# df07/mcp-raytracer

Hardware: AMD Instinct MI355X
Metric: Msamples/sec (w×h×spp/s) Cornell 800×800 spp=256 @1/2/4/8 GPU (higher is better)
Workload: dtype f64

## Files before the change

mcp-raytracer_amd/csrc/pt_kernel.hpp:

```cpp
#pragma once

#include <hip/hip_runtime.h>

#include <cstdint>
#include <type_traits>

#include "rt_math.hpp"
#include "scene.hpp"

namespace rt {

struct DevScene {
    const RtTNode* __restrict__ tnodes;
    const RtPrim* __restrict__ prims;
    const RtPrim* __restrict__ gprims;
    const RtPre* __restrict__ gpre;
    int32_t n_pre;
    const RtExact* __restrict__ xrec;
    int32_t off_xrec;
    const int32_t* __restrict__ tprims;
    const float4* __restrict__ tsph;
    const RtMat* __restrict__ mats;
    const RtLight* __restrict__ lights;
    const RtLight* __restrict__ glights;
// ... 962 lines not shown
    struct W {
        u4 a, b;
    } w{w0, w1};
    return __builtin_bit_cast(RtExact, w);
}
template <class Real>
__device__ __forceinline__ bool prim_exact_rec(const RtExact& x, const RtPrim& p, const RayK<Real>& r, Real& t) {
    const Real inf = (Real)__builtin_inf();
    const int code = x.kind & 7;
    const bool sph = code == PRE_SPHERE;
    if (code == PRE_OTHER) return prim_exact<Real>(p, r, t);
    const Real s0 = (Real)x.s0;
    Real num, den, halfB = (Real)0, sq = (Real)0;
    float o1 = 0.f, d1 = 0.f, o2 = 0.f, d2 = 0.f;
    if (sph) {
        const V3 c = V3{x.f[0], x.f[1], x.f[2]};
        const V3 oc = sub(r.o, c);
        halfB = dot<Real>(oc, r.d);
        const Real cc = len2<Real>(oc) - s0 * s0;
        const Real disc = halfB * halfB - r.a * cc;
        if (disc < (Real)0) return false;
        sq = m_sqrt(disc);
        num = -halfB - sq;
        den = r.a;
    } else {
        const int a = (int)((aquad_axes(0) >> (2 * code)) & 3u);
        const int ia = (int)((aquad_axes(1) >> (2 * code)) & 3u);
        const int ib = (int)((aquad_axes(2) >> (2 * code)) & 3u);
        const V3 o3 = r.o, d3 = r.d;
        const float oa = sel3(o3.x, o3.y, o3.z, a), da = sel3(d3.x, d3.y, d3.z, a);
        o1 = sel3(o3.x, o3.y, o3.z, ia);
        d1 = sel3(d3.x, d3.y, d3.z, ia);
        o2 = sel3(o3.x, o3.y, o3.z, ib);
        d2 = sel3(d3.x, d3.y, d3.z, ib);
        if (!(::isfinite(o1) && ::isfinite(d1) && ::isfinite(o2) && ::isfinite(d2))) return false;
        const Real na = (x.kind & kExactNegNa) ? (Real)-1 : (Real)1;
        den = na * (Real)da;
        if (m_abs(den) < (Real)1e-8) return false;
        num = s0 - na * (Real)oa;
    }
    Real q = num / den;
    if (sph) {
        if (!(K<Real>::TMIN < q && q < inf)) {
            q = (-halfB + sq) / r.a;
            if (!(K<Real>::TMIN < q && q < inf)) return false;
        }
    } else {
        if (!(K<Real>::TMIN < q && q < inf)) return false;
        const float ph1 = (o1 + (float)((Real)d1 * q)) - x.f[0];
        const float ph2 = (o2 + (float)((Real)d2 * q)) - x.f[1];
        const Real sw = (Real)x.f[2];
        const Real alpha = sw * (Real)(ph1 * x.f[3]);
        const Real beta = sw * (Real)(ph2 * x.f[4]);
        if (alpha < (Real)0 || alpha > (Real)1 || beta < (Real)0 || beta > (Real)1) return false;
    }
    t = q;
    return true;
}

constexpr float kEt = 1e-6f;
constexpr float kWin = 0.5f + 1e-4f + 1e-6f;
struct QuadPreRay {
    float c1, c0;
};
__device__ __forceinline__ QuadPreRay quad_pre_ray(const FRay& f) {
    RT_FP32_FUSED
    return QuadPreRay{(kEt + kRel) * f.dn, kRel * f.on + 1e-30f * f.dn};
}
template <int CODE>
__device__ __forceinline__ bool aquad_maybe_pre(const float* v, const FRay& f, const QuadPreRay& qr, float& lo) {
    RT_FP32_FUSED
    constexpr int a = (CODE - 1) % 3, vflag = (CODE - 1) / 3;
    constexpr int ia = vflag ? (a + 1) % 3 : (a + 2) % 3, ib = vflag ? (a + 2) % 3 : (a + 1) % 3;
    const float xa = v[0], sv = v[1], su = v[2], nq1 = v[3], nq2 = v[4], qk = v[5];
    lo = kTminLo;
    if (!(::fabsf(f.d[a]) > f.pthr)) return true;
    const float t = __builtin_fmaf(xa, f.inv[a], f.noi[a]);
    const float tn = ::fabsf(t) + ::fabsf(f.noi[a]);
    const float et = __builtin_fmaf(kEt, tn, 1e-30f);
    if (t + et < kTminLo) return false;
    lo = t - et;
    const float alpha = __builtin_fmaf(__builtin_fmaf(t, f.d[ia], f.o[ia]), sv, nq1);
    const float beta = __builtin_fmaf(__builtin_fmaf(t, f.d[ib], f.o[ib]), su, nq2);
    const float dp = __builtin_fmaf(tn, qr.c1, qr.c0 + qk);
    const float wa = __builtin_fmaf(-::fabsf(sv), dp, ::fabsf(alpha));
    const float wb = __builtin_fmaf(-::fabsf(su), dp, ::fabsf(beta));
    return !(wa > kWin) && !(wb > kWin);
}


__device__ __forceinline__ void sphere_maybe2(const float* v, const FRay& f, bool& m0, bool& m1, float& lo0,
                                              float& lo1) {
    RT_FP32_FUSED
    const pf2 cx = {v[0], v[1]}, cy = {v[2], v[3]}, cz = {v[4], v[5]}, r = {v[6], v[7]}, rr = {v[8], v[9]};
    const pf2 ox = pf2_of(f.o[0]) - cx, oy = pf2_of(f.o[1]) - cy, oz = pf2_of(f.o[2]) - cz;
    const pf2 b = pf2_fma(oz, pf2_of(f.d[2]), pf2_fma(oy, pf2_of(f.d[1]), ox * pf2_of(f.d[0])));
    const pf2 oo = pf2_fma(oz, oz, pf2_fma(oy, oy, ox * ox));
    const pf2 disc = pf2_fma(b, b, -(pf2_of(f.a) * (oo - rr)));
    const pf2 tol = pf2_fma(pf2_of(4.0f * kRel * f.a), oo + rr, pf2_of(1e-30f));
    const pf2 dt = __builtin_elementwise_max(disc, pf2_of(0.0f)) + tol;
    const pf2 sq = pf2{__builtin_amdgcn_sqrtf(dt.x), __builtin_amdgcn_sqrtf(dt.y)} * pf2_of(1.0f + kRel);
    const pf2 e0 = pf2_fma(pf2_of(3.0f), sq, pf2_fma(pf2_of(f.dn), r, pf2_of(2.0f) * pf2_abs(b)));
    const pf2 et = pf2_fma(e0, pf2_of(kRel * f.ia), pf2_of(1e-30f));
    const pf2 far = pf2_fma((sq - b) * pf2_of(f.ia), pf2_of(1.0f + kRel), et);
    const pf2 r1 = (-b - sq) * pf2_of(f.ia);
    const pf2 lo = pf2_fma(-pf2_abs(r1), pf2_of(kRel), r1) - et;
    m0 = !(disc.x < -tol.x) && !(far.x < kTminLo);
    m1 = !(disc.y < -tol.y) && !(far.y < kTminLo);
    lo0 = lo.x;
    lo1 = lo.y;
}

template <int CODE>
__device__ __forceinline__ void aquad_maybe_pre2(const float* v, const FRay& f, const QuadPreRay& qr, bool& m0,
                                                 bool& m1, float& lo0, float& lo1) {
    RT_FP32_FUSED
    constexpr int a = (CODE - 1) % 3, vflag = (CODE - 1) / 3;
    constexpr int ia = vflag ? (a + 1) % 3 : (a + 2) % 3, ib = vflag ? (a + 2) % 3 : (a + 1) % 3;
    const pf2 xa = {v[0], v[1]}, sv = {v[2], v[3]}, su = {v[4], v[5]}, nq1 = {v[6], v[7]}, nq2 = {v[8], v[9]};
    const pf2 nsv = {v[10], v[11]}, nsu = {v[12], v[13]};
    const float qk = v[14];
    const pf2 t = pf2_fma(xa, pf2_of(f.inv[a]), pf2_of(f.noi[a]));
    const float an = ::fabsf(f.noi[a]);
    const pf2 tn = {::fabsf(t.x) + an, ::fabsf(t.y) + an};
    const pf2 et = pf2_fma(pf2_of(kEt), tn, pf2_of(1e-30f));
    const pf2 te = t + et;
    const pf2 lo = t - et;
    const pf2 alpha = pf2_fma(pf2_fma(t, pf2_of(f.d[ia]), pf2_of(f.o[ia])), sv, nq1);
    const pf2 beta = pf2_fma(pf2_fma(t, pf2_of(f.d[ib]), pf2_of(f.o[ib])), su, nq2);
    const pf2 dp = pf2_fma(tn, pf2_of(qr.c1), pf2_of(qr.c0 + qk));
    const pf2 wa = pf2_fma(nsv, dp, pf2_abs(alpha));
    const pf2 wb = pf2_fma(nsu, dp, pf2_abs(beta));
    const bool par = !(::fabsf(f.d[a]) > f.pthr);
    m0 = par || (!(te.x < kTminLo) && !(wa.x > kWin) && !(wb.x > kWin));
    m1 = par || (!(te.y < kTminLo) && !(wa.y > kWin) && !(wb.y > kWin));
    lo0 = par ? kTminLo : lo.x;
    lo1 = par ? kTminLo : lo.y;
}

__device__ __forceinline__ float lot_clamp(float lo) { return lo > 0.0f ? lo : 0.0f; }
__device__ __forceinline__ uint16_t lot_store(float lo) {
    const auto h = __builtin_amdgcn_cvt_pkrtz(lot_clamp(lo), 0.0f);
    return __builtin_bit_cast(uint16_t, h[0]);
}
__device__ __forceinline__ float lot_load(uint16_t b) { return (float)__builtin_bit_cast(_Float16, b); }
template <class SK>
__device__ __forceinline__ uint16_t* lot_column(SK* stk) {
    return reinterpret_cast<uint16_t*>(stk - threadIdx.x) + threadIdx.x;
}

struct NoHook {
    __device__ void operator()() const {}
};
template <class Real, bool COUNT, class Next>
__device__ __forceinline__ int brute_nearest_first(const DevScene& S, const RayK<Real>& r, uint32_t mask, Real& t_hit,
                                                   uint32_t* cnt, Next next) {
    Real best_t = (Real)__builtin_inf();
    int best = -1;
    float thi = __builtin_inff();
    int n_exact = 0;
    if (COUNT) {
        cnt[CT_CAND0] += mask == 0u ? 1u : 0u;
        cnt[CT_CAND2] += __popc(mask) >= 2 ? 1u : 0u;
    }
    while (mask != 0u) {
        int kb;
        float lb;
        next(mask, kb, lb);
        if (lb > thi) break;
        mask &= ~(1u << kb);
        if (COUNT) {
            count_exact(cnt);
            if (++n_exact == 2) cnt[CT_EXACT2]++;
        }
        Real t;
        const bool hit = sizeof(Real) == 8
                             ? prim_exact_rec<Real>(xrec_load(S.xrec + kb), S.prims[kb], r, t)
                             : prim_exact_rec<Real>(xrec_load(S.xrec + kb), S.prims[kb], ray_at_use<Real>(r), t);
        if (hit && (t < best_t || (t == best_t && kb < best))) {
            best_t = t;
            best = kb;
            thi = upper_f<Real>(t);
        }
    }
    t_hit = best_t;
    return best;
}

template <class Real, bool COUNT>
__device__ __forceinline__ int closest_hit_primary(const DevScene& S, const RayK<Real>& r, Real& t_hit, uint2 rec,
                                                   uint32_t* cnt) {
    const int near = (int)((rec.x >> 16) & 15u);
    const float bn = lot_load((uint16_t)rec.y), bo = lot_load((uint16_t)(rec.y >> 16));
    return brute_nearest_first<Real, COUNT>(S, r, rec.x & 0xffffu, t_hit, cnt, [&](uint32_t m, int& kb, float& lb) {
        const bool n = ((m >> near) & 1u) != 0u;
        kb = n ? near : __builtin_ctz(m);
        lb = n ? bn : bo;
    });
}

template <class Real, bool COUNT, class Hook = NoHook>
__device__ __forceinline__ int closest_hit_brute_nf(const DevScene& S, int n_prims, const RayK<Real>& r, Real& t_hit,
                                                    uint16_t* lot, uint32_t* cnt, Hook after_prefilter = Hook()) {
    (void)n_prims;
    const FRay f = make_fray(r.o, r.d);
    const QuadPreRay qr = quad_pre_ray(f);
    uint32_t mask = 0u;
    for (int g = 0; g < S.n_pre; ++g) {
        const RtPre q = ld_uniform(S.gpre, g);
        const int kind = q.head & 0xff, k0 = (q.head >> 8) & 0xff, k1 = q.head >> 16;
        const float* v = q.f;
        if (kind >= PRE_SPHERE2) {
            bool m0, m1;
            float lo0, lo1;
            if (kind == PRE_SPHERE2) {
                if (COUNT) cnt[CT_SPHERE] += 2;
                sphere_maybe2(v, f, m0, m1, lo0, lo1);
            } else {
                if (COUNT) cnt[CT_QUAD] += 2;
                switch (kind - PRE_QUAD2) {
                    case 1: aquad_maybe_pre2<1>(v, f, qr, m0, m1, lo0, lo1); break;
                    case 2: aquad_maybe_pre2<2>(v, f, qr, m0, m1, lo0, lo1); break;
                    case 3: aquad_maybe_pre2<3>(v, f, qr, m0, m1, lo0, lo1); break;
                    case 4: aquad_maybe_pre2<4>(v, f, qr, m0, m1, lo0, lo1); break;
                    case 5: aquad_maybe_pre2<5>(v, f, qr, m0, m1, lo0, lo1); break;
                    default: aquad_maybe_pre2<6>(v, f, qr, m0, m1, lo0, lo1); break;
                }
            }
            const uint32_t hw = __builtin_bit_cast(uint32_t, __builtin_amdgcn_cvt_pkrtz(lot_clamp(lo0), lot_clamp(lo1)));
            if (m0) {
                lot[k0 * kStackStride] = (uint16_t)hw;
                mask |= 1u << k0;
            }
            if (m1) {
                lot[k1 * kStackStride] = (uint16_t)(hw >> 16);
                mask |= 1u << k1;
            }
            continue;
        }
        float lo;
        bool maybe;
        if (kind == PRE_SPHERE) {
            if (COUNT) cnt[CT_SPHERE]++;
            maybe = sphere_maybe(make_float4(v[0], v[1], v[2], v[3]), f, __builtin_inff(), lo);
        } else if (kind != PRE_OTHER) {
            if (COUNT) cnt[CT_QUAD]++;
            switch (kind) {
                case 1: maybe = aquad_maybe_pre<1>(v, f, qr, lo); break;
                case 2: maybe = aquad_maybe_pre<2>(v, f, qr, lo); break;
                case 3: maybe = aquad_maybe_pre<3>(v, f, qr, lo); break;
                case 4: maybe = aquad_maybe_pre<4>(v, f, qr, lo); break;
                case 5: maybe = aquad_maybe_pre<5>(v, f, qr, lo); break;
                default: maybe = aquad_maybe_pre<6>(v, f, qr, lo); break;
            }
        } else {
            maybe = prim_maybe<COUNT>(ld_uniform(S.gprims, k0), f, lo, cnt);
        }
        if (maybe) {
            lot[k0 * kStackStride] = lot_store(lo);
            mask |= 1u << k0;
        }
    }
    after_prefilter();
    return brute_nearest_first<Real, COUNT>(S, r, mask, t_hit, cnt, [&](uint32_t rest, int& kb, float& lb) {
        kb = __builtin_ctz(rest);
        lb = lot_load(lot[kb * kStackStride]);
        for (uint32_t m = rest & (rest - 1u); m != 0u; m &= m - 1u) {
            const int k = __builtin_ctz(m);
            const float l = lot_load(lot[k * kStackStride]);
            if (l < lb) {
                lb = l;
                kb = k;
            }
        }
    });
}

struct Onb {
    V3 u, v, w;
};
template <class Real>
__device__ __forceinline__ Onb make_onb(V3 n) {
    Onb b;
    b.w = unit<Real>(n);
    const V3 a = m_abs((Real)b.w.x) > (Real)0.9 ? v3(0, 1, 0) : v3(1, 0, 0);
    b.v = unit<Real>(cross<Real>(b.w, a));
    b.u = cross<Real>(b.w, b.v);
    return b;
}
template <class Real>
__device__ __forceinline__ V3 onb_local(const Onb& b, V3 a) {
    return add(add(scale<Real>(b.u, (Real)a.x), scale<Real>(b.v, (Real)a.y)), scale<Real>(b.w, (Real)a.z));
}

template <class Real>
__device__ __forceinline__ V3 random_in_unit_sphere(uint64_t& rng) {
    while (true) {
        const Real x = (Real)-1 + (Real)2 * uniform<Real>(rng);
        const Real y = (Real)-1 + (Real)2 * uniform<Real>(rng);
        const Real z = (Real)-1 + (Real)2 * uniform<Real>(rng);
        const V3 p = mk<Real>(x, y, z);
        if (len2<Real>(p) < (Real)1) return p;
    }
}

template <class Real>
__device__ __forceinline__ V3 dielectric_dir(Real ior, bool front, V3 din, V3 n, uint64_t& rng, bool& reflected) {
    const Real ratio = front ? ((Real)1 / ior) : ior;
    const V3 ud = unit<Real>(din);
    const Real cosT = js_min<Real>(dot<Real>(neg(ud), n), (Real)1);
    const Real sinT = m_sqrt((Real)1 - cosT * cosT);
    const bool cannot = ratio * sinT > (Real)1;
    bool refl = cannot;
    if (!refl) {
        Real r0 = ((Real)1 - ratio) / ((Real)1 + ratio);
        r0 = r0 * r0;
        const Real reflectance = r0 + ((Real)1 - r0) * pow5((Real)1 - cosT);
        refl = reflectance > uniform<Real>(rng);
    }
    reflected = refl;
    if (refl) return reflect<Real>(ud, n);
    const V3 perp = scale<Real>(add(ud, scale<Real>(n, cosT)), ratio);
    const V3 par = scale<Real>(n, -m_sqrt(m_abs((Real)1 - len2<Real>(perp))));
    return add(perp, par);
}

enum ScatterKind { SC_NONE = 0, SC_SPEC = 1, SC_PDF = 2 };

template <class Real>
__device__ __forceinline__ int scatter(const DevScene& S, int mi, V3 din, V3 n, bool front, uint64_t& rng, V3& att,
                                       V3& dir, int* pdf_mat = nullptr) {
    while (true) {
        const RtMat m = S.mats[mi];
        switch (m.type) {
            case MAT_LAMBERT:
                att = ld3(m.color);
                if (pdf_mat) *pdf_mat = mi;
                return SC_PDF;
            case MAT_METAL: {
                const V3 refl = reflect<Real>(unit<Real>(din), n);
                const Real fuzz = (Real)m.p0;
                V3 f = refl;
                if (fuzz > (Real)0) f = add(refl, scale<Real>(random_in_unit_sphere<Real>(rng), fuzz));
                if (dot<Real>(f, n) <= (Real)0) return SC_NONE;
                att = ld3(m.color);
                dir = f;
                return SC_SPEC;
            }
            case MAT_GLASS: {
                bool r;
                dir = dielectric_dir<Real>((Real)m.p0, front, din, n, rng, r);
                att = v3(1, 1, 1);
                return SC_SPEC;
            }
            case MAT_MIXED:
                mi = uniform<Real>(rng) < (Real)m.p0 ? m.c0 : m.c1;
                continue;
            case MAT_LAYERED: {
                bool r;
                const V3 d2 = dielectric_dir<Real>((Real)S.mats[m.c0].p0, front, din, n, rng, r);
                if (r) {
                    att = v3(1, 1, 1);
                    dir = d2;
                    return SC_SPEC;
                }
                din = d2;
                mi = m.c1;
                continue;
            }
            default:
                return SC_NONE;
        }
    }
}

template <class Real, bool COUNT, bool UNIFORM = false>
__device__ __forceinline__ Real light_pdf_value(const DevScene& S, const RtLight& L, V3 origin, V3 dir,
                                                uint32_t* cnt) {
    const RtPrim p = UNIFORM ? ld_uniform(S.gprims, L.prim) : S.prims[L.prim];
    const RayK<Real> r = make_ray<Real>(origin, dir);
    Real t;
    if (L.type == PRIM_QUAD) {
        if (COUNT) cnt[CT_LIGHT_QUAD]++;
        const int code = aquad_code(p);
        const bool hit = code != 0 ? aquad_t<Real>(p, code, origin, dir, K<Real>::TMIN, (Real)__builtin_inf(), t)
                                   : planar_t<Real, true>(p, r, K<Real>::TMIN, (Real)__builtin_inf(), t);
        if (!hit) return (Real)0;
        const V3 hp = ray_at<Real>(origin, dir, t);
        const V3 n = ld3(p.g3);
        const bool front = dot<Real>(dir, n) <= (Real)0;
        const V3 hn = front ? n : neg(n);
        const Real d2 = len2<Real>(sub(hp, origin));
        const Real cosine = m_abs(dot<Real>(dir, hn));
        return d2 / ((Real)L.area * cosine);
    }
    if (COUNT) cnt[CT_LIGHT_SPHERE]++;
    if (!sphere_t<Real>(p, r, K<Real>::TMIN, (Real)__builtin_inf(), t)) return (Real)0;
    const Real rad = sphere_radius<Real>(p);
    const Real d2 = len2<Real>(sub(ld3(p.g0), origin));
    if (d2 <= rad * rad) return (Real)1 / ((Real)4 * K<Real>::PI);
    const Real cosT = m_sqrt((Real)1 - rad * rad / d2);
    const Real solid = (Real)2 * K<Real>::PI * ((Real)1 - cosT);
    return (Real)1 / solid;
}

template <class Real>
__device__ __forceinline__ V3 light_generate(const DevScene& S, const RtLight& L, V3 origin, uint64_t& rng) {
    const RtPrim p = S.prims[L.prim];
    if (L.type == PRIM_QUAD) {
        const Real alpha = uniform<Real>(rng);
        const Real beta = uniform<Real>(rng);
        const V3 rp = add(add(ld3(p.g0), scale<Real>(ld3(p.g1), alpha)), scale<Real>(ld3(p.g2), beta));
        return unit<Real>(sub(rp, origin));
    }
    const V3 oc = sub(ld3(p.g0), origin);
    const Real d2 = len2<Real>(oc);
    const Onb b = make_onb<Real>(oc);
    const Real rad = sphere_radius<Real>(p);
    const Real r1 = uniform<Real>(rng);
    const Real r2 = uniform<Real>(rng);
    const Real z = (Real)1 + r2 * (m_sqrt((Real)1 - rad * rad / d2) - (Real)1);
    const Real phi = (Real)2 * K<Real>::PI * r1;
    const Real s = m_sqrt((Real)1 - z * z);
    Real sn, cs;
    m_sincos(phi, sn, cs);
    return onb_local<Real>(b, mk<Real>(cs * s, sn * s, z));
}

__device__ __forceinline__ double div_pi(double x) {
    constexpr double kPi = 3.141592653589793, kInvPi = 1.0 / 3.141592653589793;
    const double q = x * kInvPi;
    const double r = __builtin_fma(-q, kPi, x);
    return __builtin_fma(r, kInvPi, q);
}
__device__ __forceinline__ float div_pi(float x) { return x / K<float>::PI; }

template <class Real>
__device__ __forceinline__ Real cosine_value(const Onb& b, V3 dir) {
    const Real c = dot<Real>(unit<Real>(dir), b.w);
    return c <= (Real)0 ? (Real)0 : div_pi(c);
}

__device__ __forceinline__ uint8_t to_u8(float c) {
    const double r = ::sqrt((double)c);
    const double v = ::floor(255.999 * r);
    if (!(v > 0.0)) return 0;
    if (v >= 255.0) return 255;
    return (uint8_t)v;
}

__device__ __forceinline__ unsigned long long wave_sum(unsigned long long v) {
#pragma unroll
    for (int o = 32; o > 0; o >>= 1) v += __shfl_xor(v, o, 64);
    return v;
}
__device__ __forceinline__ unsigned long long wave_min(unsigned long long v) {
#pragma unroll
    for (int o = 32; o > 0; o >>= 1) { unsigned long long x = __shfl_xor(v, o, 64); v = x < v ? x : v; }
    return v;
}
__device__ __forceinline__ unsigned long long wave_max(unsigned long long v) {
#pragma unroll
    for (int o = 32; o > 0; o >>= 1) { unsigned long long x = __shfl_xor(v, o, 64); v = x > v ? x : v; }
    return v;
}

__device__ __forceinline__ bool pixel_converged_at_batch(const RtCamera& c, int n, double sIll, double sIll2);
__device__ __forceinline__ bool pixel_converged(const RtCamera& c, int n, double sIll, double sIll2) {
    if (c.a_tolerance <= 0.0 || c.samples <= 1.0 || n < 2) return false;
    const double rem = ::fmod((double)n, c.a_batch);
    if (rem != 0.0) return false;
    return pixel_converged_at_batch(c, n, sIll, sIll2);
}
__device__ __forceinline__ bool pixel_converged_at_batch(const RtCamera& c, int n, double sIll, double sIll2) {
    if (c.a_tolerance <= 0.0 || c.samples <= 1.0 || n < 2) return false;
    const double mean = sIll / n;
    const double var = (sIll2 - (sIll * sIll) / n) / (n - 1);
    if (var <= 0.0 || var != var) return true;
    const double ci = 1.96 * ::sqrt(var) / ::sqrt((double)n);
    return ci <= c.a_tolerance * mean;
}

typedef const __attribute__((address_space(4))) char* KArgPtr;
__device__ __forceinline__ const RtCamera& cam_opaque() {
    KArgPtr p = (KArgPtr)__builtin_amdgcn_kernarg_segment_ptr();
    asm volatile("" : "+s"(p));
    return *(const RtCamera*)(p + offsetof(DevScene, cam));
}

template <class Real, bool COUNT, int TRAV, class SK>
__device__ __forceinline__ int closest_hit_any(const DevScene& S, int n_prims, const RayK<Real>& r, Real& t, SK* stk,
                                               uint32_t* cnt) {
    if (TRAV == TRAV_BRUTE) {
        if (n_prims <= kBruteMaxPrims)
            return closest_hit_brute_nf<Real, COUNT>(S, n_prims, r, t, lot_column(stk), cnt);
        return closest_hit_brute<Real, COUNT>(S, n_prims, r, t, cnt);
    }
    if (trav_fast(TRAV)) return closest_hit_fast<Real, COUNT, TRAV == TRAV_FAST_DEFER>(S, r, t, stk, cnt);
    return closest_hit<Real, COUNT>(S, r, t, stk, cnt);
}

__device__ __forceinline__ unsigned long long clk() { return __builtin_amdgcn_s_memtime(); }

constexpr int kProfSlot = 2 + 3 * PR_WORDS;
constexpr int kProfWaves = 16;
struct Prof {
    unsigned long long* w;
};
template <bool PROF>
__device__ __forceinline__ void prof_init(Prof& pf, unsigned long long* lds, int lane) {
    if (PROF) {
        pf.w = lds + (threadIdx.x >> 6) * kProfSlot;
        if (lane == 0) {
            for (int k = 0; k < kProfSlot; ++k) pf.w[k] = 0ull;
            const unsigned long long n = __builtin_amdgcn_s_memtime();
            pf.w[0] = n;
            pf.w[1] = n;
        }
    }
}
template <bool PROF>
__device__ __forceinline__ void psec(Prof& pf, int k) {
    if (PROF) {
        const unsigned long long m = __ballot(1);
        if ((int)(threadIdx.x & 63) == __builtin_ctzll(m)) {
            const unsigned long long n = __builtin_amdgcn_s_memtime();
            pf.w[2 + k] += n - pf.w[0];
            pf.w[0] = n;
            pf.w[2 + PR_WORDS + k] += (unsigned long long)__popcll(m);
            pf.w[2 + 2 * PR_WORDS + k] += 1ull;
        }
    }
}
template <bool PROF>
__device__ __forceinline__ void pcount(Prof& pf, int k) {
    if (PROF) {
        const unsigned long long m = __ballot(1);
        if ((int)(threadIdx.x & 63) == __builtin_ctzll(m)) {
            pf.w[2 + PR_WORDS + k] += (unsigned long long)__popcll(m);
            pf.w[2 + 2 * PR_WORDS + k] += 1ull;
        }
    }
}
template <bool PROF>
__device__ __forceinline__ void prof_trip(Prof& pf) {
    if (PROF) {
        const unsigned long long m = __ballot(1);
        if ((int)(threadIdx.x & 63) == __builtin_ctzll(m)) pf.w[2 + PR_TRIPS] += 1ull;
    }
}

template <bool EMIT>
struct Path {
    uint64_t rng;
    V3 o, d, T;
    int bounces;
    int em_n;
    V3 em[EMIT ? kEmitStack : 1];
};

template <class Real>
__device__ __forceinline__ V3 pixel_center(const RtCamera& C, int i, int j) {
    return add(add(ld3(C.pixel00), scale<float>(ld3(C.du), (float)i)), scale<float>(ld3(C.dv), (float)j));
}

template <class Real, bool EMIT>
__device__ __forceinline__ void path_begin(const RtCamera& C, Path<EMIT>& P, V3 pc, uint32_t pix, uint32_t sample) {
    P.rng = rng_init(C.seed_mix, pix, sample);
    const V3 du = ld3(C.du), dv = ld3(C.dv), cen = ld3(C.center);
    V3 ps = pc;
    if (C.samples > 1.0) {
        const Real px = (Real)-0.5 + uniform<Real>(P.rng);
        const Real py = (Real)-0.5 + uniform<Real>(P.rng);
        ps = add(add(pc, scale<Real>(du, px)), scale<Real>(dv, py));
    }
    P.o = cen;
    P.d = sub(ps, cen);
    if (C.aperture > 0.0) {
        V3 rd;
        while (true) {
            const Real a = (Real)2 * uniform<Real>(P.rng) - (Real)1;
            const Real b = (Real)2 * uniform<Real>(P.rng) - (Real)1;
            rd = mk<Real>(a, b, (Real)0);
            if (len2<Real>(rd) < (Real)1) break;
        }
        const V3 off = add(scale<Real>(ld3(C.ddu), (Real)rd.x), scale<Real>(ld3(C.ddv), (Real)rd.y));
        P.o = add(cen, off);
        P.d = sub(ps, P.o);
    }
    P.T = v3(1, 1, 1);
    P.bounces = 0;
    P.em_n = 0;
}

template <bool EMIT>
__device__ __forceinline__ void fold_emission(const Path<EMIT>& P, V3& c) {
    if (EMIT) {
        for (int k = min(P.em_n, kEmitStack) - 1; k >= 0; --k) c = add(P.em[k], c);
    }
}

template <class Real, bool EMIT, bool PROF>
__device__ __forceinline__ bool path_pre(const RtCamera& C, Path<EMIT>& P, Prof& pf, V3& c) {
    bool term = false;
    c = v3(0, 0, 0);
    if (P.bounces >= C.depth) {
        term = true;
    } else if (C.roulette && P.bounces >= C.roulette_depth) {
        const Real mc = js_max<Real>(js_max<Real>((Real)P.T.x, (Real)P.T.y), (Real)P.T.z);
        const Real p = js_min<Real>(mc, (Real)0.95);
        if (uniform<Real>(P.rng) > p) term = true;
        else P.T = divs<Real>(P.T, p);
    }
    if (term) fold_emission<EMIT>(P, c);
    psec<PROF>(pf, PR_RR);
    return term;
}


template <class Real, bool EMIT, bool PROF>
__device__ __forceinline__ V3 miss_color(const RtCamera& C, const Path<EMIT>& P, unsigned long long& st_err,
                                         Prof& pf) {
    if (!C.has_background) st_err |= ERR_NO_BACKGROUND;
    const V3 ud = unit<Real>(P.d);
    const Real a = (Real)0.5 * ((Real)ud.y + (Real)1);
    const V3 c = mulv(add(scale<Real>(ld3(C.bg_top), (Real)1 - a), scale<Real>(ld3(C.bg_bottom), a)), P.T);
    psec<PROF>(pf, PR_MISS);
    return c;
}

template <class Real, bool EMIT, bool COUNT, bool PROF>
__device__ __forceinline__ int shade_hit(const DevScene& S, Path<EMIT>& P, int h, Real t, uint32_t* cnt, Prof& pf,
                                         V3& p, V3& nrm, bool& front, bool& planar, V3& emitted, V3& att, V3& sdir,
                                         int* pdf_mat = nullptr) {
    if (COUNT) cnt[CT_MATERIAL]++;
    const RtPrim pr = S.prims[h];
    p = ray_at<Real>(P.o, P.d, t);
    planar = pr.type != PRIM_SPHERE;
    if (!planar) {
        nrm = scale<Real>(sub(p, ld3(pr.g0)), sphere_inv_radius<Real>(pr));
        front = dot<Real>(P.d, nrm) <= (Real)0;
        if (!front) nrm = neg(nrm);
    } else {
        const V3 pn = ld3(pr.g3);
        front = dot<Real>(P.d, pn) <= (Real)0;
        nrm = front ? pn : neg(pn);
    }
    const RtMat hm = S.mats[pr.mat];
    emitted = mulv(ld3(hm.emitted), P.T);
    psec<PROF>(pf, PR_HITREC);
    const int kind = scatter<Real>(S, pr.mat, P.d, nrm, front, P.rng, att, sdir, pdf_mat);
    psec<PROF>(pf, PR_SCATTER);
    return kind;
}

template <class Real, bool EMIT, bool COUNT, bool PROF, int BR = 0>
__device__ __forceinline__ bool shade_diffuse(const DevScene& S, const RtCamera& C, Path<EMIT>& P, int h, bool planar,
                                              bool front, V3 p, V3 nrm, V3 att, uint32_t* cnt, Prof& pf) {
    if (COUNT) cnt[CT_DIFFUSE]++;
    Onb b;
    if (planar && h < S.n_onb) {
        const RtOnb& ob = S.onbs[(h * 2 + (sizeof(Real) == 4 ? 1 : 0)) * 2 + (front ? 0 : 1)];
        if (BR != 2) {
            b.u = ld3(ob.u);
            b.v = ld3(ob.v);
        }
        b.w = ld3(ob.w);
    } else if (BR == 2) {
        b.w = unit<Real>(nrm);
    } else {
        b = make_onb<Real>(nrm);
    }
    const Real total = (Real)S.mix_total;
    const bool total1 = S.mix_total == 1.0;
    const Real lw = (Real)S.light_w;
    const Real u0 = uniform<Real>(P.rng);
    const Real rnd = total1 ? u0 : u0 * total;
    Real partial = (Real)0.5;
    V3 gdir;
    if (BR == 1 || (BR == 0 && (rnd < partial || C.n_lights == 0))) {
        const Real r1 = uniform<Real>(P.rng);
        const Real r2 = uniform<Real>(P.rng);
        const Real phi = (Real)2 * K<Real>::PI * r1;
        const Real sr2 = m_sqrt(r2);
        Real sn, cs;
        m_sincos(phi, sn, cs);
        gdir = onb_local<Real>(b, mk<Real>(cs * sr2, sn * sr2, m_sqrt((Real)1 - r2)));
    } else {
        int pick = C.n_lights - 1;
        for (int l = 0; l < C.n_lights; ++l) {
            partial += lw;
            if (rnd < partial) { pick = l; break; }
        }
        gdir = light_generate<Real>(S, S.lights[pick], p, P.rng);
    }
    psec<PROF>(pf, PR_SAMPLE);
    const Real cv = cosine_value<Real>(b, gdir);
    Real sum = (Real)0.5 * cv;
    for (int l = 0; l < C.n_lights; ++l)
        sum += lw * light_pdf_value<Real, COUNT, true>(S, ld_uniform(S.glights, l), p, gdir, cnt);
    const Real pv = total1 ? sum : sum / total;
    bool term = false;
    if (pv <= (Real)0.0001) {
        term = true;
    } else {
        const V3 brdf = scale<Real>(att, cv);
        P.T = divs<Real>(mulv(P.T, brdf), pv);
        P.o = p;
        P.d = gdir;
    }
    psec<PROF>(pf, PR_PDF);
    return term;
}

template <class Real, bool EMIT, bool COUNT, bool PROF>
__device__ __forceinline__ bool path_post(const DevScene& S, const RtCamera& C, Path<EMIT>& P, int h, Real t,
                                          uint32_t* cnt, unsigned long long& st_err, Prof& pf, V3& c) {
    bool term = false;
    c = v3(0, 0, 0);
    if (h < 0) {
        term = true;
        c = miss_color<Real, EMIT, PROF>(C, P, st_err, pf);
    } else {
        V3 p, nrm, emitted, att, sdir;
        bool front, planar;
        const int kind = shade_hit<Real, EMIT, COUNT, PROF>(S, P, h, t, cnt, pf, p, nrm, front, planar, emitted, att,
                                                            sdir);
        if (kind == SC_NONE) {
            term = true;
            c = emitted;
        } else {
            ++P.bounces;
            if (kind == SC_SPEC) {
                P.T = mulv(P.T, att);
                P.o = p;
                P.d = sdir;
            } else if (shade_diffuse<Real, EMIT, COUNT, PROF>(S, C, P, h, planar, front, p, nrm, att, cnt, pf)) {
                term = true;
                c = emitted;
            }
            if (EMIT && !term) {
                if (P.em_n < kEmitStack) P.em[P.em_n] = emitted;
                else st_err |= ERR_EMIT_STACK;
                ++P.em_n;
            }
        }
    }
    if (term) fold_emission<EMIT>(P, c);
    return term;
}

template <class Real, bool EMIT, bool COUNT, bool PROF, int TRAV, class SK>
__device__ __forceinline__ bool path_trip(const DevScene& S, const RtCamera& C, Path<EMIT>& P, SK* stk, uint32_t* cnt,
                                          unsigned long long& st_err, Prof& pf, V3& c) {
    if (path_pre<Real, EMIT, PROF>(C, P, pf, c)) return true;
    const RayK<Real> ray = make_ray<Real>(P.o, P.d);
    Real t;
    if (COUNT) cnt[CT_RAYS]++;
    const int h = closest_hit_any<Real, COUNT, TRAV>(S, C.n_prims, ray, t, stk, cnt);
    psec<PROF>(pf, PR_HIT);
    return path_post<Real, EMIT, COUNT, PROF>(S, C, P, h, t, cnt, st_err, pf, c);
}

struct PixStats {
    unsigned long long pixels = 0, samples = 0, smin = ~0ull, smax = 0, b = 0, bmin = ~0ull, bmax = 0;
};
__device__ __forceinline__ void finish_pixel(const RtCamera& C, const RenderOut& out, uint32_t opix, V3 color, int n,
                                             unsigned long long bsum, int bmin, int bmax, PixStats& st) {
    V3 fin;
    if (C.mode == MODE_BOUNCES) {
        const double avg = n > 0 ? (double)bsum / (double)n : 0.0;
        fin = mk<double>(0.0, 0.0, js_min<double>(avg / (double)C.depth_raw, 1.0));
    } else if (C.mode == MODE_SAMPLES) {
        fin = mk<double>(js_min<double>((double)n / C.samples, 1.0), 0.0, 0.0);
    } else {
        fin = divs<double>(color, (double)n);
    }
    const size_t off = (size_t)opix * 3;
    if (out.radiance) {
        out.radiance[off] = fin.x;
        out.radiance[off + 1] = fin.y;
        out.radiance[off + 2] = fin.z;
    }
    if (out.rgb) {
        out.rgb[off] = to_u8(fin.x);
        out.rgb[off + 1] = to_u8(fin.y);
        out.rgb[off + 2] = to_u8(fin.z);
    }
    if (out.px_samples) out.px_samples[opix] = n;
    if (out.px_bounces) out.px_bounces[opix] = (int32_t)bsum;
    st.pixels += 1;
    st.samples += (unsigned long long)n;
    st.smin = min(st.smin, (unsigned long long)n);
    st.smax = max(st.smax, (unsigned long long)n);
    st.b += bsum;
    if (n > 0) st.bmin = min(st.bmin, (unsigned long long)bmin);
    st.bmax = max(st.bmax, (unsigned long long)bmax);
}

__device__ __forceinline__ void stats_atomics(const RenderOut& out, unsigned long long sp, unsigned long long ss,
                                              unsigned long long smn, unsigned long long smx, unsigned long long sb,
                                              unsigned long long bmn, unsigned long long bmx, unsigned long long err) {
    unsigned long long* w = out.stats;
    if (sp > 0) {
        atomicAdd(&w[ST_PIXELS * kStatStride], sp);
        atomicAdd(&w[ST_SAMPLES * kStatStride], ss);
        atomicMin(&w[ST_SMIN * kStatStride], smn);
        atomicMax(&w[ST_SMAX * kStatStride], smx);
    }
    if (sp > 0 || bmn != ~0ull) {
        atomicAdd(&w[ST_BOUNCES * kStatStride], sb);
        atomicMin(&w[ST_BMIN * kStatStride], bmn);
        atomicMax(&w[ST_BMAX * kStatStride], bmx);
    }
    if (err) atomicOr(&w[ST_ERROR * kStatStride], err);
}
__device__ __forceinline__ unsigned long long wave_or(unsigned long long v) {
#pragma unroll
    for (int k = 32; k > 0; k >>= 1) v |= __shfl_xor(v, k, 64);
    return v;
}
__device__ __forceinline__ void publish_stats(const RenderOut& out, const PixStats& st, unsigned long long st_err,
                                              int lane) {
    const unsigned long long sp = wave_sum(st.pixels), ss = wave_sum(st.samples), sb = wave_sum(st.b);
    const unsigned long long smn = wave_min(st.smin), smx = wave_max(st.smax);
    const unsigned long long bmn = wave_min(st.bmin), bmx = wave_max(st.bmax);
    const unsigned long long err = wave_or(st_err);
    if (lane == 0) stats_atomics(out, sp, ss, smn, smx, sb, bmn, bmx, err);
}

template <bool COUNT, bool PROF>
__device__ __forceinline__ void publish_counters(const RenderOut& out, const uint32_t* cnt, Prof& pf, int lane) {
    if (COUNT) {
#pragma unroll
        for (int k = 0; k < CT_WORDS; ++k) {
            const unsigned long long v = wave_sum((unsigned long long)cnt[k]);
            if (lane == 0 && v) atomicAdd(&out.counters[k], v);
        }
    }
    if (PROF) {
        psec<PROF>(pf, PR_TILE);
        if (lane == 0) {
            const unsigned long long life = __builtin_amdgcn_s_memtime() - pf.w[1];
            for (int k = 0; k < PR_WORDS; ++k)
                atomicAdd(&out.counters[CT_WORDS + k], k == PR_LOOP ? life : pf.w[2 + k]);
            for (int k = 0; k < PR_LOOP; ++k) {
                atomicAdd(&out.counters[CT_WORDS + PR_WORDS + k], pf.w[2 + PR_WORDS + k]);
                atomicAdd(&out.counters[CT_WORDS + PR_WORDS + PR_LOOP + k], pf.w[2 + 2 * PR_WORDS + k]);
            }
        }
    }
}

// ... 435 lines not shown
                else slot = -1;
                psec<PROF>(pf, PR_ACC);
            }
        }
    }
    PixStats st;
    lb.to(st);
    publish_stats(out, st, st_err, lane);
    publish_counters<COUNT, PROF>(out, cnt, pf, lane);
#undef PK_SB
#undef PK_REG
#undef PK_OUT
#undef PK_S
}

#ifndef RT_POOL_K
#define RT_POOL_K 152
#endif
#ifndef RT_POOL_PROF
#define RT_POOL_PROF 0
#endif
constexpr int kPoolK = RT_POOL_K;
constexpr int kBlockPool = 1024;
constexpr int kPoolGroups = 3;
static_assert(kPoolK >= kWave && kPoolK <= 256, "pool slots: one full wave, u8 queue entries");
constexpr size_t kPoolWaveBytes = ((size_t)kPoolK * (kPoolGroups * 16 + 8) + 2 * kPoolK + 15) / 16 * 16;
constexpr int kPoolClog2Bits = 3;
constexpr int kPoolMaxChunk = 1 << ((1 << kPoolClog2Bits) - 1);
__device__ __forceinline__ float pool_meta(int phase, int clog2, int mat) {
    return __uint_as_float((uint32_t)((phase + 2) & 0xff) | ((uint32_t)clog2 << 8) | ((uint32_t)mat << 11));
}
__device__ __forceinline__ int meta_phase(float m) { return (int)(__float_as_uint(m) & 0xffu) - 2; }
__device__ __forceinline__ int meta_clog2(float m) { return (int)((__float_as_uint(m) >> 8) & 7u); }
__device__ __forceinline__ int meta_mat(float m) { return (int)(__float_as_uint(m) >> 11); }
__device__ __forceinline__ float pool_hs(int hf16, int s) { return __uint_as_float(((uint32_t)hf16 & 0xffffu) | ((uint32_t)s << 16)); }
__device__ __forceinline__ int hs_s(float v) { return (int)(__float_as_uint(v) >> 16); }
__device__ __forceinline__ int hs_hf(float v) { return (int)(__float_as_uint(v) & 0xffffu); }
__device__ __forceinline__ int item_end(int s, int clog2) { return ((s >> clog2) + 1) << clog2; }
constexpr size_t pool_lds_bytes() { return (size_t)(kBlockPool / kWave) * kPoolWaveBytes; }
enum : int { PH_NEW = -1, PH_ITEM = -2 };

__device__ __forceinline__ void stack_push(uint8_t* q, bool top, int& cnt, bool want, int k) {
    const unsigned long long m = __ballot(want);
    if (want) {
        const int r = __builtin_amdgcn_mbcnt_hi((uint32_t)(m >> 32), __builtin_amdgcn_mbcnt_lo((uint32_t)m, 0u));
        q[top ? kPoolK - 1 - (cnt + r) : cnt + r] = (uint8_t)k;
    }
    cnt += __popcll(m);
}

struct KernArgsPrimary {
    KernArgs args;
    const uint2* ptab;
};
__device__ __forceinline__ const uint2* primary_table_opaque() {
    KArgPtr p = (KArgPtr)__builtin_amdgcn_kernarg_segment_ptr();
    asm volatile("" : "+s"(p));
    return *(const uint2* const*)(p + offsetof(KernArgsPrimary, ptab));
}

template <class Real, int TRAV, int LDSS, bool PRIM>
__device__ __forceinline__ void pool_trips(DevScene S0, RtRegion reg, RenderOut out, int tiles_x, SampleBuf sb) {
    extern __shared__ int lds_stack[];
    const RtCamera& C0 = S0.cam;
    __shared__ PhaseRow ptab[kMaxPhases];
    phase_table_init(sb, ptab);
    const DevScene S = scene_prologue<LDSS>(S0, lds_stack);
    const int lane = threadIdx.x & (kWave - 1);
    StackT<LDSS>* stk = reinterpret_cast<StackT<LDSS>*>(lds_stack) + threadIdx.x;
    char* wpool = reinterpret_cast<char*>(lds_stack) + S0.lds_pool_off + (size_t)(threadIdx.x / kWave) * kPoolWaveBytes;
    float4* G = reinterpret_cast<float4*>(wpool);
    float2* G3 = reinterpret_cast<float2*>(wpool + (size_t)kPoolK * kPoolGroups * 16);
    uint8_t* qa = reinterpret_cast<uint8_t*>(wpool + (size_t)kPoolK * (kPoolGroups * 16 + 8));
    uint8_t* qd = qa + kPoolK;
    const int endX = min(reg.x + reg.width, C0.width);
    const int endY = min(reg.y + reg.height, C0.height);
    const int n_items = sb.n_items;
    const double rtx = 1.0 / (double)tiles_x;
    uint32_t* cnt = nullptr;
    unsigned long long st_err = 0;
    constexpr bool PP = RT_POOL_PROF;
    __shared__ unsigned long long prof_lds[PP ? kProfWaves * kProfSlot : 1];
    Prof pf;
    prof_init<PP>(pf, prof_lds, lane);

    for (int k = lane; k < kPoolK; k += kWave) {
        qa[k] = (uint8_t)k;
        G[k] = make_float4(0.f, 0.f, pool_meta(PH_ITEM, 0, 0), 0.f);
    }
    int d_cnt = 0, dl_cnt = 0;
    int an_cnt = kPoolK, ac_cnt = 0;
    int pool_next, pool_end;
    bool exhausted;
    first_pool(sb, pool_next, pool_end, exhausted);

    LaneBounces lb;
    auto record = [&](V3 c, int bounces, int slot, int& s, int s_end, unsigned long long err = 0ull) -> int {
        if (!sb.err_in_rec) st_err |= err;
        rec_put<true>(sb, (size_t)s * sb.stride_s + (size_t)slot * sb.stride_slot, c,
                           bounces | (sb.err_in_rec ? (int)((uint32_t)err << kRecErrShift) : 0), lb, out.stats);
        ++s;
        return s < s_end ? PH_NEW : PH_ITEM;
    };

    enum : int { FR_N, FR_D, FR_NONE };
    while (an_cnt + ac_cnt + d_cnt + dl_cnt > 0) {
        __asm__ volatile("" ::: "memory");
        prof_trip<PP>(pf);
        psec<PP>(pf, PR_ACC);
        const bool dtop = dl_cnt > d_cnt;
        const int dn = dtop ? dl_cnt : d_cnt;
        const int fr = dn >= kWave       ? FR_D
                       : ac_cnt >= kWave ? FR_NONE
                       : an_cnt >= kWave ? FR_N
                       : dn > 0          ? FR_D
                       : an_cnt > 0      ? FR_N
                                         : FR_NONE;
        int k = -1;
        int nd = 0;
        if (fr == FR_D) {
            nd = min(kWave, dn);
            const int na = min(kWave - nd, ac_cnt);
            if (lane < nd) k = (int)qd[dtop ? kPoolK - dl_cnt + lane : d_cnt - nd + lane];
            else if (lane < nd + na) k = (int)qa[kPoolK - ac_cnt + lane - nd];
            if (dtop) dl_cnt -= nd;
            else d_cnt -= nd;
            ac_cnt -= na;
        } else if (fr == FR_N) {
            const int n = min(kWave, an_cnt);
            if (lane < n) k = (int)qa[an_cnt - n + lane];
            an_cnt -= n;
        } else {
            const int n = min(kWave, ac_cnt);
            if (lane < n) k = (int)qa[kPoolK - ac_cnt + lane];
            ac_cnt -= n;
        }
        float4 g0 = make_float4(0.f, 0.f, pool_meta(PH_ITEM, 0, 0), 0.f), g1 = g0, g2 = g0;
        float2 g3 = make_float2(0.f, 0.f);
        if (k >= 0) {
            g0 = G[k];
            g1 = G[kPoolK + k];
            g2 = G[2 * kPoolK + k];
            g3 = G3[k];
        }
        int phase = meta_phase(g0.z), clog2 = meta_clog2(g0.z), slot = __float_as_int(g1.w);
        int s = hs_s(g0.w);
        const RtCamera& C = cam_opaque();
        Path<false> P;
        bool keep = k >= 0;
        bool path = false;
        bool term = false;
        V3 c = v3(0, 0, 0);
        uint2 prec = make_uint2(0u, 0u);
        if (fr == FR_N) {
            const unsigned long long need = __ballot(k >= 0 && phase == PH_ITEM);
            if (need != 0ull && !exhausted) {
                if (pool_next >= pool_end) take_pool(out, sb, lane, pool_next, pool_end, exhausted);
                if (!exhausted) {
                    const int take = min(__popcll(need), pool_end - pool_next);
                    const int rank = __builtin_amdgcn_mbcnt_hi((uint32_t)(need >> 32),
                                                               __builtin_amdgcn_mbcnt_lo((uint32_t)need, 0u));
                    if (k >= 0 && phase == PH_ITEM && rank < take) {
                        int tl, l, s1, e1, i, j;
                        item_decode(sb, ptab, pool_next + rank, tl, l, s1, e1);
                        if (slot_pixel(sb, reg, tiles_x, rtx, endX, endY, tl * 64 + l, i, j)) {
                            slot = tl * 64 + l;
                            s = s1;
                            clog2 = __builtin_ctz((uint32_t)(e1 - s1));
                            phase = PH_NEW;
                        }
                    }
                    pool_next += take;
                }
            }
            keep = k >= 0 && (phase != PH_ITEM || !exhausted);
            if (k >= 0 && phase == PH_NEW) {
                path = true;
                int i, j;
                slot_pixel(sb, reg, tiles_x, rtx, endX, endY, slot, i, j);
                const uint32_t pix = (uint32_t)j * (uint32_t)C.width + (uint32_t)i;
                if (PRIM) prec = primary_table_opaque()[pix];
                path_begin<Real, false>(C, P, pixel_center<Real>(C, i, j), pix, (uint32_t)(sb.s_base + s));
                if (PRIM) __builtin_amdgcn_s_waitcnt(0x0F70);
            }
            psec<PP>(pf, PR_NEWPATH);
        } else {
            if (k >= 0) {
                path = true;
                P.rng = (uint64_t)__float_as_uint(g0.x) | ((uint64_t)__float_as_uint(g0.y) << 32);
                P.o = V3{g1.x, g1.y, g1.z};
                P.d = V3{g2.x, g2.y, g2.z};
                P.T = V3{g2.w, g3.x, g3.y};
                P.bounces = phase;
                P.em_n = 0;
            }
            if (fr == FR_D) {
                if (lane < nd) {
                    const int hf = hs_hf(g0.w);
                    const int h = hf & 0x3fff;
                    const bool planar = (hf >> 14) & 1, front = (hf >> 15) & 1;
                    const V3 att = ld3(S.mats[meta_mat(g0.z)].color);
                    const bool dterm =
                        dtop ? shade_diffuse<Real, false, false, PP, 2>(S, C, P, h, planar, front, P.o, P.d, att, cnt, pf)
                             : shade_diffuse<Real, false, false, PP, 1>(S, C, P, h, planar, front, P.o, P.d, att, cnt, pf);
                    if (dterm) {
                        term = true;
                        c = mulv(ld3(S.mats[S.prims[h].mat].emitted), P.T);
                    }
                }
            } else {
                psec<PP>(pf, PR_NEWPATH);
            }
        }
        bool to_d = false, d_light = false;
        int hf = 0, dmat = 0;
        unsigned long long err = 0ull;
        if (path && !term) {
            term = path_pre<Real, false, PP>(C, P, pf, c);
            if (!term) {
                const RayK<Real> ray = make_ray<Real>(P.o, P.d);
                Real t;
                int h;
                V3 att;
                if (PRIM && fr == FR_N) {
                    psec<PP>(pf, PR_TILE);
                    h = closest_hit_primary<Real, false>(S, ray, t, prec, cnt);
                } else if (PP && TRAV == TRAV_BRUTE && C.n_prims <= kBruteMaxPrims)
                    h = closest_hit_brute_nf<Real, false>(S, C.n_prims, ray, t, lot_column(stk), cnt,
                                                          [&]() { psec<PP>(pf, PR_TILE); });
                else
                    h = closest_hit_any<Real, false, TRAV>(S, C.n_prims, ray, t, stk, cnt);
                psec<PP>(pf, PR_HIT);
                if (h < 0) {
                    term = true;
                    c = miss_color<Real, false, PP>(C, P, err, pf);
                } else {
                    V3 p, nrm, emitted, sdir;
                    bool front, planar;
                    const int kind = shade_hit<Real, false, false, PP>(S, P, h, t, cnt, pf, p, nrm, front, planar,
                                                                          emitted, att, sdir, &dmat);
                    if (kind == SC_NONE) {
                        term = true;
                        c = emitted;
                    } else {
                        ++P.bounces;
                        P.o = p;
                        if (kind == SC_SPEC) {
                            P.T = mulv(P.T, att);
                            P.d = sdir;
                        } else {
                            to_d = true;
                            P.d = nrm;
                            hf = h | (planar ? (1 << 14) : 0) | (front ? (1 << 15) : 0);
                            {
                                uint64_t r = P.rng;
                                const Real u0 = uniform<Real>(r);
                                const Real rnd = S.mix_total == 1.0 ? u0 : u0 * (Real)S.mix_total;
                                d_light = !(rnd < (Real)0.5 || C.n_lights == 0);
                            }
                        }
                    }
                }
            }
        }
        if (path) {
            phase = term ? record(c, P.bounces, slot, s, item_end(s, clog2), err) : P.bounces;
            g0 = make_float4(__uint_as_float((uint32_t)P.rng), __uint_as_float((uint32_t)(P.rng >> 32)),
                             pool_meta(phase, clog2, to_d ? dmat : 0), pool_hs(to_d ? hf : 0, s));
            g1 = make_float4(P.o.x, P.o.y, P.o.z, __int_as_float(slot));
            g2 = make_float4(P.d.x, P.d.y, P.d.z, P.T.x);
            g3 = make_float2(P.T.y, P.T.z);
        } else if (keep) {
            g0 = make_float4(0.f, 0.f, pool_meta(PH_ITEM, 0, 0), 0.f);
        }
        if (keep) {
            G[k] = g0;
            G[kPoolK + k] = g1;
            G[2 * kPoolK + k] = g2;
            G3[k] = g3;
        }
        stack_push(qa, false, an_cnt, keep && !to_d && phase < 0, k);
        stack_push(qa, true, ac_cnt, keep && !to_d && phase >= 0, k);
        stack_push(qd, false, d_cnt, to_d && !d_light, k);
        stack_push(qd, true, dl_cnt, to_d && d_light, k);
    }
    PixStats st;
    lb.to(st);
    publish_stats(out, st, st_err, lane);
    publish_counters<false, PP>(out, cnt, pf, lane);
}

template <class Real, int TRAV, int LDSS>
__global__ __launch_bounds__(kBlockPool) void pt_pool_kernel(DevScene S0, RtRegion reg, RenderOut out, int tiles_x,
                                                               SampleBuf sb) {
    pool_trips<Real, TRAV, LDSS, false>(S0, reg, out, tiles_x, sb);
}
template <class Real, int TRAV, int LDSS>
__global__ __launch_bounds__(kBlockPool) void pt_pool_primary_kernel(DevScene S0, RtRegion reg, RenderOut out,
                                                                       int tiles_x, SampleBuf sb, const uint2* ptab) {
    (void)ptab;
    pool_trips<Real, TRAV, LDSS, true>(S0, reg, out, tiles_x, sb);
}

}
```

Measured before the change: 13770.

## Reuse light-PDF intersection results to seed brute-force closest-hit search

When evaluating the light PDF for the sampled diffuse direction, the exact light-primitive intersection is recorded in a HitSeed (mask of known prims plus best t). The following closest-hit brute search starts from that seed, tightening its initial upper bound and removing already-tested light prims from the candidate mask. This avoids recomputing exact f64 intersections with lights along the continuation ray. It adds register pressure, plumbing through several functions, and a wave-uniform readfirstlane of the known mask that assumes all lanes test the same lights.

```diff
diff --git a/mcp-raytracer_amd/csrc/pt_kernel.hpp b/mcp-raytracer_amd/csrc/pt_kernel.hpp
--- a/mcp-raytracer_amd/csrc/pt_kernel.hpp
+++ b/mcp-raytracer_amd/csrc/pt_kernel.hpp
@@ -1138,12 +1138,26 @@
 struct NoHook {
     __device__ void operator()() const {}
 };
+template <class Real>
+struct HitSeed {
+    Real t = (Real)__builtin_inf();
+    int best = -1;
+    uint32_t known = 0u;
+    __device__ __forceinline__ void add(int slot, bool hit, Real th) {
+        known |= 1u << (slot & 31);
+        if (hit && (th < t || (th == t && slot < best))) {
+            t = th;
+            best = slot;
+        }
+    }
+};
+
 template <class Real, bool COUNT, class Next>
 __device__ __forceinline__ int brute_nearest_first(const DevScene& S, const RayK<Real>& r, uint32_t mask, Real& t_hit,
-                                                   uint32_t* cnt, Next next) {
-    Real best_t = (Real)__builtin_inf();
-    int best = -1;
-    float thi = __builtin_inff();
+                                                   uint32_t* cnt, Next next, HitSeed<Real> seed = HitSeed<Real>()) {
+    Real best_t = seed.t;
+    int best = seed.best;
+    float thi = seed.best >= 0 ? upper_f<Real>(seed.t) : __builtin_inff();
     int n_exact = 0;
     if (COUNT) {
         cnt[CT_CAND0] += mask == 0u ? 1u : 0u;
@@ -1187,7 +1201,9 @@
 
 template <class Real, bool COUNT, class Hook = NoHook>
 __device__ __forceinline__ int closest_hit_brute_nf(const DevScene& S, int n_prims, const RayK<Real>& r, Real& t_hit,
-                                                    uint16_t* lot, uint32_t* cnt, Hook after_prefilter = Hook()) {
+                                                    uint16_t* lot, uint32_t* cnt,
+                                                    HitSeed<Real> seed = HitSeed<Real>(),
+                                                    Hook after_prefilter = Hook()) {
     (void)n_prims;
     const FRay f = make_fray(r.o, r.d);
     const QuadPreRay qr = quad_pre_ray(f);
@@ -1248,6 +1264,7 @@
         }
     }
     after_prefilter();
+    mask &= ~seed.known;
     return brute_nearest_first<Real, COUNT>(S, r, mask, t_hit, cnt, [&](uint32_t rest, int& kb, float& lb) {
         kb = __builtin_ctz(rest);
         lb = lot_load(lot[kb * kStackStride]);
@@ -1259,7 +1276,7 @@
                 kb = k;
             }
         }
-    });
+    }, seed);
 }
 
 struct Onb {
@@ -1362,7 +1379,7 @@
 
 template <class Real, bool COUNT, bool UNIFORM = false>
 __device__ __forceinline__ Real light_pdf_value(const DevScene& S, const RtLight& L, V3 origin, V3 dir,
-                                                uint32_t* cnt) {
+                                                uint32_t* cnt, HitSeed<Real>* seed = nullptr) {
     const RtPrim p = UNIFORM ? ld_uniform(S.gprims, L.prim) : S.prims[L.prim];
     const RayK<Real> r = make_ray<Real>(origin, dir);
     Real t;
@@ -1371,6 +1388,7 @@
         const int code = aquad_code(p);
         const bool hit = code != 0 ? aquad_t<Real>(p, code, origin, dir, K<Real>::TMIN, (Real)__builtin_inf(), t)
                                    : planar_t<Real, true>(p, r, K<Real>::TMIN, (Real)__builtin_inf(), t);
+        if (seed) seed->add(L.prim, hit, t);
         if (!hit) return (Real)0;
         const V3 hp = ray_at<Real>(origin, dir, t);
         const V3 n = ld3(p.g3);
@@ -1381,7 +1399,9 @@
         return d2 / ((Real)L.area * cosine);
     }
     if (COUNT) cnt[CT_LIGHT_SPHERE]++;
-    if (!sphere_t<Real>(p, r, K<Real>::TMIN, (Real)__builtin_inf(), t)) return (Real)0;
+    const bool hit = sphere_t<Real>(p, r, K<Real>::TMIN, (Real)__builtin_inf(), t);
+    if (seed) seed->add(L.prim, hit, t);
+    if (!hit) return (Real)0;
     const Real rad = sphere_radius<Real>(p);
     const Real d2 = len2<Real>(sub(ld3(p.g0), origin));
     if (d2 <= rad * rad) return (Real)1 / ((Real)4 * K<Real>::PI);
@@ -1476,10 +1496,10 @@
 
 template <class Real, bool COUNT, int TRAV, class SK>
 __device__ __forceinline__ int closest_hit_any(const DevScene& S, int n_prims, const RayK<Real>& r, Real& t, SK* stk,
-                                               uint32_t* cnt) {
+                                               uint32_t* cnt, HitSeed<Real> seed = HitSeed<Real>()) {
     if (TRAV == TRAV_BRUTE) {
         if (n_prims <= kBruteMaxPrims)
-            return closest_hit_brute_nf<Real, COUNT>(S, n_prims, r, t, lot_column(stk), cnt);
+            return closest_hit_brute_nf<Real, COUNT>(S, n_prims, r, t, lot_column(stk), cnt, seed);
         return closest_hit_brute<Real, COUNT>(S, n_prims, r, t, cnt);
     }
     if (trav_fast(TRAV)) return closest_hit_fast<Real, COUNT, TRAV == TRAV_FAST_DEFER>(S, r, t, stk, cnt);
@@ -1642,7 +1662,8 @@
 
 template <class Real, bool EMIT, bool COUNT, bool PROF, int BR = 0>
 __device__ __forceinline__ bool shade_diffuse(const DevScene& S, const RtCamera& C, Path<EMIT>& P, int h, bool planar,
-                                              bool front, V3 p, V3 nrm, V3 att, uint32_t* cnt, Prof& pf) {
+                                              bool front, V3 p, V3 nrm, V3 att, uint32_t* cnt, Prof& pf,
+                                              HitSeed<Real>* seed = nullptr) {
     if (COUNT) cnt[CT_DIFFUSE]++;
     Onb b;
     if (planar && h < S.n_onb) {
@@ -1684,7 +1705,7 @@
     const Real cv = cosine_value<Real>(b, gdir);
     Real sum = (Real)0.5 * cv;
     for (int l = 0; l < C.n_lights; ++l)
-        sum += lw * light_pdf_value<Real, COUNT, true>(S, ld_uniform(S.glights, l), p, gdir, cnt);
+        sum += lw * light_pdf_value<Real, COUNT, true>(S, ld_uniform(S.glights, l), p, gdir, cnt, seed);
     const Real pv = total1 ? sum : sum / total;
     bool term = false;
     if (pv <= (Real)0.0001) {
@@ -2426,6 +2447,9 @@
         bool term = false;
         V3 c = v3(0, 0, 0);
         uint2 prec = make_uint2(0u, 0u);
+        constexpr bool SEED = sizeof(Real) == 8 && TRAV == TRAV_BRUTE;
+        HitSeed<Real> seed;
+        uint32_t lights = 0u;
         if (fr == FR_N) {
             const unsigned long long need = __ballot(k >= 0 && phase == PH_ITEM);
             if (need != 0ull && !exhausted) {
@@ -2474,14 +2498,17 @@
                     const int h = hf & 0x3fff;
                     const bool planar = (hf >> 14) & 1, front = (hf >> 15) & 1;
                     const V3 att = ld3(S.mats[meta_mat(g0.z)].color);
-                    const bool dterm =
-                        dtop ? shade_diffuse<Real, false, false, PP, 2>(S, C, P, h, planar, front, P.o, P.d, att, cnt, pf)
-                             : shade_diffuse<Real, false, false, PP, 1>(S, C, P, h, planar, front, P.o, P.d, att, cnt, pf);
+                    HitSeed<Real>* const sd = SEED ? &seed : nullptr;
+                    const bool dterm = dtop ? shade_diffuse<Real, false, false, PP, 2>(S, C, P, h, planar, front, P.o,
+                                                                                        P.d, att, cnt, pf, sd)
+                                            : shade_diffuse<Real, false, false, PP, 1>(S, C, P, h, planar, front, P.o,
+                                                                                        P.d, att, cnt, pf, sd);
                     if (dterm) {
                         term = true;
                         c = mulv(ld3(S.mats[S.prims[h].mat].emitted), P.T);
                     }
                 }
+                if (SEED) lights = __builtin_amdgcn_readfirstlane(seed.known);
             } else {
                 psec<PP>(pf, PR_NEWPATH);
             }
@@ -2496,14 +2523,15 @@
                 Real t;
                 int h;
                 V3 att;
+                if (SEED) seed.known = lane < nd ? lights : 0u;
                 if (PRIM && fr == FR_N) {
                     psec<PP>(pf, PR_TILE);
                     h = closest_hit_primary<Real, false>(S, ray, t, prec, cnt);
                 } else if (PP && TRAV == TRAV_BRUTE && C.n_prims <= kBruteMaxPrims)
-                    h = closest_hit_brute_nf<Real, false>(S, C.n_prims, ray, t, lot_column(stk), cnt,
+                    h = closest_hit_brute_nf<Real, false>(S, C.n_prims, ray, t, lot_column(stk), cnt, seed,
                                                           [&]() { psec<PP>(pf, PR_TILE); });
                 else
-                    h = closest_hit_any<Real, false, TRAV>(S, C.n_prims, ray, t, stk, cnt);
+                    h = closest_hit_any<Real, false, TRAV>(S, C.n_prims, ray, t, stk, cnt, seed);
                 psec<PP>(pf, PR_HIT);
                 if (h < 0) {
                     term = true;
```

Result: no change. 13910 (median of 6 runs) (+1.0%).
